# AY-Liu/Image-Editing-Framework

Hardware: AMD Instinct MI355X
Metric: denoising steps/sec (SD1.5 512x512 P2P edit step, UNet batch 4) (higher is better)
Workload: dtype f16x3; 1 GPU; sd15 UNet (859.5M params) P2P AttentionRefine edit step, 2 prompts x CFG = batch 4, 64x64 latents (512x512 px), 50-step DDIM, guidance 7.5, cross 0.8 / self 0.4, per-step null-text unconditional embeddings (P2P_NTI, edit_real.py); one independent edit per GPU; precision mode f16x3: fp32 storage; every contraction on split operands: hi + lo fp16 halves of each fp32 element, Ah Bh + Al Bh + Ah Bl =

## Files before the change

### image-editing-framework_amd/csrc/conv_halo_x3p.hip

```cpp
#include "x3p_common.h"

template <int N>
struct IntTag { static constexpr int value = N; };

template <bool UPS>
__global__ __launch_bounds__(768) void conv3x3_halo_x3p_kernel(const IefGemmX3pParams p) {
    constexpr int BM = 256, BN = 80, BK = XP_BK, NW = 8, NL = 4;
    constexpr int TM = 2, TN = 5;
    constexpr int WMAX = 64;
    constexpr int NPA = (BM + 2 * WMAX + 2 + 15) / 16;
    constexpr int APL = NPA * 1024;
    constexpr int AD = 2 * APL + 128;
    constexpr int ZA = 2 * APL;
    constexpr int NPB = BN / 16;
    constexpr int BPL = NPB * 1024, BBUF = 2 * BPL, NSB = 5;
    constexpr int BOFF = 2 * AD, DUMP = BOFF + NSB * BBUF;
    constexpr int LDS_BYTES = DUMP + 1024;
    constexpr int NU = 2 * NPA;
    constexpr int ATAPS = 5, APT = 3;
    static_assert(ATAPS * APT * NL >= NU && 3 * NL >= 2 * NPB, "loader schedule");
    static_assert(LDS_BYTES <= 160 * 1024, "LDS");
    __shared__ __attribute__((aligned(1024))) char smem[LDS_BYTES];

    const int tid = threadIdx.x, lane = tid & 63;
    const int wave = __builtin_amdgcn_readfirstlane(tid >> 6);
    const int tiles_n = (p.N + BN - 1) / BN, tiles_m = (p.M + BM - 1) / BM;
    const int lid = xcd_remap(blockIdx.x, gridDim.x);
    const int grp = lid / (XP_GROUP_M * tiles_n), within = lid - grp * (XP_GROUP_M * tiles_n);
    const int gsz = min(XP_GROUP_M, tiles_m - grp * XP_GROUP_M);
    const int tn = within / gsz, tm = grp * XP_GROUP_M + (within - tn * gsz);
    const int m0 = tm * BM, n0 = tn * BN;
    const int W = p.Wd, H = p.H;
    const int Ctot = p.C1 + p.C2;
    const char* __restrict__ zp = (const char*)p.zeros;
    const int Wi = W >> 1, Hi = H >> 1;
    const int ups_img = m0 / (H * W), ups_y0 = (m0 - ups_img * H * W) / W;
    const int ups_rel = ((ups_y0 - 1) >> 1) * Wi - 1;
    const int src_pixels = UPS ? p.batch_images * Hi * Wi : p.M;
    const int st_row0 = UPS ? ups_img * Hi * Wi + ups_rel : m0 - (W + 1);

    const int ncb = Ctot / BK;
    int cb_lo = 0, cb_hi = ncb;
    if (p.splits > 1) {
        const int per = (ncb + p.splits - 1) / p.splits;
        cb_lo = min(ncb, (int)blockIdx.y * per);
        cb_hi = min(ncb, cb_lo + per);
    }
    const int nblk = cb_hi - cb_lo, nsteps = nblk * 9;

    if (tid < 16) { ((float*)(smem + ZA))[tid] = 0.f; ((float*)(smem + ZA + AD))[tid] = 0.f; }
    asm volatile("s_waitcnt lgkmcnt(0)" ::: "memory");

    if (wave >= NW) {
        const int l = wave - NW;
        bool abl_prologue = true;
        const unsigned st_chunk = (unsigned)(XP_LANE_CHUNK(lane) * 16);
        const int ms_lane = st_row0 + (lane >> 2);
        const char* an_src = zp; long long an_pl = 0; unsigned an_cs = 0, an_c0 = 0; bool an_on = false;
        auto set_next_block = [&](int cb, bool on) {
            const bool first = cb * BK < p.C1;
            an_src = (const char*)(first ? p.A : p.A2);
            an_pl = (first ? p.planeA : p.planeA2) * 2;
            an_cs = (unsigned)(first ? p.C1 : p.C2);
            an_c0 = (unsigned)(first ? cb * BK : cb * BK - p.C1);
            an_on = on;
        };
        auto issue_a = [&](int u, int buf_off) {
            const bool exists = u < NU;
            const int pl = u >= NPA ? 1 : 0, q = u - pl * NPA;
            const int ms = ms_lane + 16 * q;
            const bool ok = exists && an_on && (unsigned)ms < (unsigned)src_pixels;
            const char* g = ok ? an_src + ((long long)pl * an_pl + (long long)((unsigned)ms * an_cs + an_c0) * 2 + st_chunk) : zp;
            if (!(XP_ABL & 1) || abl_prologue) glds16(g, (half_t*)(smem + (exists ? pl * AD + buf_off + q * 1024 : DUMP)));
        };
        const long long w_lane = (long long)(n0 + (lane >> 2)) * p.K * 2 + st_chunk;
        auto issue_b = [&](int cb, int tap, bool on, int slot_off) {
            const long long k0 = (long long)(tap * Ctot + cb * BK) * 2;
#pragma unroll
            for (int j = 0; j < 3; ++j) {
                const int v = l + NL * j;
                const bool exists = v < 2 * NPB;
                const int pl = v >= NPB ? 1 : 0, q = v - pl * NPB;
                const bool ok = exists && on && n0 + 16 * q + (lane >> 2) < p.N;
                const char* g = ok ? (const char*)p.W + ((long long)pl * p.planeW * 2 + w_lane + (long long)(16 * q) * p.K * 2 + k0) : zp;
                if (!(XP_ABL & 1) || abl_prologue) glds16(g, (half_t*)(smem + (exists ? BOFF + slot_off + pl * BPL + q * 1024 : DUMP)));
            }
        };
        auto n_issued = [](int tap) constexpr -> int { return 3 + (tap < ATAPS ? APT : 0); };
        if (nsteps > 0) {
            set_next_block(cb_lo, true);
            for (int u = l; u < ((NU + NL - 1) / NL) * NL; u += NL) issue_a(u, 0);
            issue_b(cb_lo, 0, true, 0);
            issue_b(cb_lo, 1, nsteps > 1, BBUF);
            issue_b(cb_lo, 2, nsteps > 2, 2 * BBUF);
            issue_b(cb_lo, 3, nsteps > 3, 3 * BBUF);
            asm volatile("s_waitcnt vmcnt(9)" ::: "memory");
            XP_BARRIER();
        }
        abl_prologue = false;
        int bs_prev = 4 * BBUF, bs = 0, bs_next = BBUF;
        for (int cbi = 0; cbi < nblk; ++cbi) {
            const int cb = cb_lo + cbi;
            const int abuf_n = APL - (cbi & 1) * APL;
            set_next_block(min(cb + 1, cb_hi - 1), cb + 1 < cb_hi);
            const int steps_left = nsteps - cbi * 9;
            auto one_step = [&](auto tap_tag) {
                constexpr int tap = decltype(tap_tag)::value;
                if (!(XP_ABL & 1)) asm volatile("s_waitcnt vmcnt(%0)" ::"n"(n_issued((tap + 8) % 9) + n_issued((tap + 7) % 9)) : "memory");
                XP_BARRIER();
                if constexpr (tap < ATAPS) {
#pragma unroll
                    for (int j = 0; j < APT; ++j) issue_a(APT * NL * tap + l + NL * j, abuf_n);
                }
                issue_b(cb + (tap + 4) / 9, (tap + 4) % 9, tap + 4 < steps_left, bs_prev);
                bs_prev = bs; bs = bs_next; bs_next = bs_next == (NSB - 1) * BBUF ? 0 : bs_next + BBUF;
            };
            one_step(IntTag<0>{}); one_step(IntTag<1>{}); one_step(IntTag<2>{});
            one_step(IntTag<3>{}); one_step(IntTag<4>{}); one_step(IntTag<5>{});
            one_step(IntTag<6>{}); one_step(IntTag<7>{}); one_step(IntTag<8>{});
        }
        asm volatile("s_waitcnt vmcnt(0)" ::: "memory");
        return;
    }

    const int fr = lane & 15, fq = lane >> 4;
    int a_row[TM], a_x[TM], a_y[TM];
    unsigned a_edge[TM];
#pragma unroll
    for (int i = 0; i < TM; ++i) {
        const int r = wave * 32 + i * 16 + fr, m = m0 + r;
        const int x = m % W, y = (m / W) % H;
        a_row[i] = r; a_x[i] = x; a_y[i] = y;
        a_edge[i] = (x == 0 ? 1u : 0u) | (x == W - 1 ? 2u : 0u) | (y == 0 ? 4u : 0u) | (y == H - 1 ? 8u : 0u) | (m >= p.M ? 16u : 0u);
    }
    int b_off[TN];
#pragma unroll
    for (int j = 0; j < TN; ++j) {
        const int row = j * 16 + fr;
        b_off[j] = BOFF + row * 64 + ((fq ^ xp_swz(row)) << 4);
    }
    f32x4 acc[TN][TM];
#pragma unroll
    for (int j = 0; j < TN; ++j)
#pragma unroll
        for (int i = 0; i < TM; ++i) acc[j][i] = f32x4{0.f, 0.f, 0.f, 0.f};

    auto a_addr = [&](int i, int abuf, int ky, int kx) -> int {
        const unsigned tmask = 16u | (kx == 0 ? 1u : 0u) | (kx == 2 ? 2u : 0u) | (ky == 0 ? 4u : 0u) | (ky == 2 ? 8u : 0u);
        int sr;
        if constexpr (UPS) sr = ((a_y[i] + ky - 1) >> 1) * Wi + ((a_x[i] + kx - 1) >> 1) - ups_rel;
        else sr = a_row[i] + ky * W + kx;
        const int ad = abuf + sr * 64 + ((fq ^ xp_swz(sr)) << 4);
        return (a_edge[i] & tmask) ? ZA : ad;
    };
    half8 ah[2][TM], al[2][TM], bh[TN], bl[TN];
    bool abl_read_done = false;
    auto read_a = [&](half8 (&h)[TM], half8 (&l)[TM], int abuf, int ky, int kx) {
        if ((XP_ABL & 2) && abl_read_done) return;
#pragma unroll
        for (int i = 0; i < TM; ++i) {
            const int ad = a_addr(i, abuf, ky, kx);
            h[i] = *(const half8*)(smem + ad);
            l[i] = *(const half8*)(smem + ad + AD);
        }
    };
    if (nsteps > 0) {
        XP_BARRIER();
        read_a(ah[0], al[0], 0, 0, 0);
#pragma unroll
        for (int j = 0; j < TN; ++j) { bh[j] = *(const half8*)(smem + b_off[j]); bl[j] = *(const half8*)(smem + b_off[j] + BPL); }
    }
    int bs_next = BBUF;
    auto one_step = [&](auto tap_tag, auto par_tag, int abuf, int abuf_n) {
        constexpr int tap = decltype(tap_tag)::value, PAR = decltype(par_tag)::value;
        XP_BARRIER();
        {
            constexpr int nky = tap == 8 ? 0 : (tap + 1) / 3, nkx = tap == 8 ? 0 : (tap + 1) % 3;
            read_a(ah[PAR ^ 1], al[PAR ^ 1], tap == 8 ? abuf_n : abuf, nky, nkx);
        }
#pragma unroll
        for (int j = 0; j < TN; ++j) {
#pragma unroll
            for (int i = 0; i < TM; ++i) {
                if (!(XP_ABL & 4)) {
                    acc[j][i] = __builtin_amdgcn_mfma_f32_16x16x32_f16(bl[j], ah[PAR][i], acc[j][i], 0, 0, 0);
                    acc[j][i] = __builtin_amdgcn_mfma_f32_16x16x32_f16(bh[j], al[PAR][i], acc[j][i], 0, 0, 0);
                }
                acc[j][i] = __builtin_amdgcn_mfma_f32_16x16x32_f16(bh[j], ah[PAR][i], acc[j][i], 0, 0, 0);
            }
            if (!(XP_ABL & 2)) {
                bh[j] = *(const half8*)(smem + bs_next + b_off[j]);
                bl[j] = *(const half8*)(smem + bs_next + b_off[j] + BPL);
            }
        }
        abl_read_done = true;
        bs_next = bs_next == (NSB - 1) * BBUF ? 0 : bs_next + BBUF;
    };
    for (int cbi = 0; cbi < nblk; cbi += 2) {
        {
            const int abuf = 0, abuf_n = APL;
            one_step(IntTag<0>{}, IntTag<0>{}, abuf, abuf_n); one_step(IntTag<1>{}, IntTag<1>{}, abuf, abuf_n);
            one_step(IntTag<2>{}, IntTag<0>{}, abuf, abuf_n); one_step(IntTag<3>{}, IntTag<1>{}, abuf, abuf_n);
            one_step(IntTag<4>{}, IntTag<0>{}, abuf, abuf_n); one_step(IntTag<5>{}, IntTag<1>{}, abuf, abuf_n);
            one_step(IntTag<6>{}, IntTag<0>{}, abuf, abuf_n); one_step(IntTag<7>{}, IntTag<1>{}, abuf, abuf_n);
            one_step(IntTag<8>{}, IntTag<0>{}, abuf, abuf_n);
        }
        if (cbi + 1 < nblk) {
            const int abuf = APL, abuf_n = 0;
            one_step(IntTag<0>{}, IntTag<1>{}, abuf, abuf_n); one_step(IntTag<1>{}, IntTag<0>{}, abuf, abuf_n);
            one_step(IntTag<2>{}, IntTag<1>{}, abuf, abuf_n); one_step(IntTag<3>{}, IntTag<0>{}, abuf, abuf_n);
            one_step(IntTag<4>{}, IntTag<1>{}, abuf, abuf_n); one_step(IntTag<5>{}, IntTag<0>{}, abuf, abuf_n);
            one_step(IntTag<6>{}, IntTag<1>{}, abuf, abuf_n); one_step(IntTag<7>{}, IntTag<0>{}, abuf, abuf_n);
            one_step(IntTag<8>{}, IntTag<1>{}, abuf, abuf_n);
        }
    }
    asm volatile("s_waitcnt lgkmcnt(0)" ::: "memory");

    const float inv = p.inv_scale;
    if (p.splits > 1) {
        float* slab = p.ws + (long long)blockIdx.y * p.M * p.N;
#pragma unroll
        for (int i = 0; i < TM; ++i) {
            const int m = m0 + wave * 32 + i * 16 + fr;
            if (m >= p.M) continue;
#pragma unroll
            for (int j = 0; j < TN; ++j) {
                const int n = n0 + j * 16 + 4 * fq;
                if (n < p.N) *(f32x4*)(slab + (long long)m * p.N + n) = acc[j][i] * inv;
            }
        }
        return;
    }
#pragma unroll
    for (int i = 0; i < TM; ++i) {
        const int m = m0 + wave * 32 + i * 16 + fr;
        if (m >= p.M) continue;
#pragma unroll
        for (int j = 0; j < TN; ++j) {
            const int n = n0 + j * 16 + 4 * fq;
            if (n < p.N) xp_store(p, acc[j][i] * inv, m, n);
        }
    }
}

int ief_conv_halo_x3p_dispatch(const IefGemmX3pParams& p, hipStream_t st) {
    if (!p.conv || p.stride != 1 || p.pad_hi_only || p.CE1 || p.CE2 || p.Wd < 2 || p.H < 2 || p.geglu) return IEF_ESHAPE;
    if (p.ups) {
        if (p.tile != 12 || p.Wd > 128 || (p.H * p.Wd) % 256 || 256 % p.Wd) return IEF_ESHAPE;
    } else if (p.tile != 11 || p.Wd > 64) return IEF_ESHAPE;
    const int ncb = (p.C1 + p.C2) / XP_BK;
    if (p.splits > ncb) return IEF_ESHAPE;
    const int tiles = ((p.M + 255) / 256) * ((p.N + 79) / 80);
    const int splits = p.splits > 1 ? p.splits : 1;
    if (p.ups) hipLaunchKernelGGL(conv3x3_halo_x3p_kernel<true>, dim3(tiles, splits), dim3(768), 0, st, p);
    else hipLaunchKernelGGL(conv3x3_halo_x3p_kernel<false>, dim3(tiles, splits), dim3(768), 0, st, p);
    IEF_LAUNCH_CHECK();
    return IEF_OK;
}
```

### image-editing-framework_amd/csrc/gemm_x3p.hip

```cpp
#include "ief_common.h"
#include "ief_params.h"
#include "x3_common.h"

#include "x3p_common.h"

template <int BM, int BN, int WAVES_M, int WAVES_N, int NS, int NL, bool CONV>
__global__ __launch_bounds__(64 * (WAVES_M * WAVES_N + NL)) void igemm_x3p_kernel(const IefGemmX3pParams p) {
    constexpr int BK = XP_BK;
    constexpr int NWC = WAVES_M * WAVES_N;
    constexpr int NSW = NL > 0 ? NL : NWC;
    constexpr int PA = BM / 16, PB = BN / 16;
    constexpr int P = 2 * (PA + PB);
    constexpr int G = (P + NSW - 1) / NSW;
    constexpr int WM = BM / WAVES_M, WN = BN / WAVES_N, TM = WM / 16, TN = WN / 16;
    constexpr int SLOT = P * 16 * BK;
    constexpr int DUMP = NS * SLOT;
    static_assert(BM % 16 == 0 && BN % 16 == 0 && WM % 16 == 0 && WN % 16 == 0, "tile");
    static_assert(NS >= 2 && NS <= 4, "ring depth");
    static_assert((NS * SLOT + 512) * 2 <= 160 * 1024, "LDS");
    __shared__ __attribute__((aligned(1024))) half_t smem[NS * SLOT + 512];

    const int tid = threadIdx.x, lane = tid & 63;
    const int wave = __builtin_amdgcn_readfirstlane(tid >> 6);
    const int wr = wave / WAVES_N, wc = wave % WAVES_N;
// ... 320 lines not shown
                }
            }
        }
        return;
    }
    const int slots_out = (p.N + WN - 1) / WN;
#pragma unroll
    for (int i = 0; i < TM; ++i) {
        const int m = m0 + wr * WM + i * 16 + fr;
        const bool mok = m < p.M;
        float mu = 0.f, rs = 1.f;
        if (p.rstat_in && mok) xp_ln_row(p, m, mu, rs);
        f32x4 vv[TN];
#pragma unroll
        for (int j = 0; j < TN; ++j) vv[j] = f32x4{0.f, 0.f, 0.f, 0.f};
#pragma unroll
        for (int P = 0; P < NP2; ++P) {
            const int n = cb + 32 * P + 8 * fq;
            if (!mok || n >= p.N) continue;
            f32x4 v0 = acc[2 * P][i] * inv, v1 = acc[2 * P + 1][i] * inv;
            if (n + 4 < p.N) {
                if (p.rstat_in) {
                    v0 = (v0 - *(const f32x4*)(p.colsum + n) * mu) * rs;
                    v1 = (v1 - *(const f32x4*)(p.colsum + n + 4) * mu) * rs;
                }
                xp_store8(p, v0, v1, m, n);
                vv[2 * P] = v0; vv[2 * P + 1] = v1;
            } else {
                if (p.rstat_in) v0 = (v0 - *(const f32x4*)(p.colsum + n) * mu) * rs;
                vv[2 * P] = xp_store(p, v0, m, n);
            }
        }
        if constexpr (TN & 1) {
            constexpr int j = TN - 1;
            const int n = cb + j * 16 + 4 * fq;
            if (mok && n < p.N) {
                f32x4 v = acc[j][i] * inv;
                if (p.rstat_in) v = (v - *(const f32x4*)(p.colsum + n) * mu) * rs;
                vv[j] = xp_store(p, v, m, n);
            }
        }
        if (p.rstat_out) {
            float sm, sq;
            xp_row_stats<TN>(vv, sm, sq);
            if (fq == 0 && mok && cb < p.N) {
                float* ro = p.rstat_out + ((long long)m * slots_out + cb / WN) * 2;
                ro[0] = sm; ro[1] = sq;
            }
        }
    }
}

__global__ __launch_bounds__(256) void x3p_reduce_kernel(const IefGemmX3pParams p) {
    const int N4 = p.N >> 2;
    const long long total = (long long)p.M * N4, slab = (long long)p.M * p.N;
    for (long long i = (long long)blockIdx.x * 256 + threadIdx.x; i < total; i += (long long)gridDim.x * 256) {
        const int m = (int)(i / N4), n = (int)(i - (long long)m * N4) * 4;
        const float* w = p.ws + (long long)m * p.N + n;
        f32x4 a = *(const f32x4*)w;
        int s = 1;
        for (; s + 3 < p.splits; s += 4) {
            f32x4 t[4];
#pragma unroll
            for (int u = 0; u < 4; ++u) t[u] = *(const f32x4*)(w + (s + u) * slab);
#pragma unroll
            for (int u = 0; u < 4; ++u) a += t[u];
        }
        for (; s < p.splits; ++s) a += *(const f32x4*)(w + s * slab);
        xp_store(p, a, m, n);
    }
}

__global__ __launch_bounds__(256) void x3_split_act_kernel(const float* __restrict__ x, half_t* __restrict__ planes, long long plane,
                                                           long long rows, int C4, int ldx, int ldp, float scale) {
    const long long total = rows * C4;
    for (long long i = (long long)blockIdx.x * 256 + threadIdx.x; i < total; i += (long long)gridDim.x * 256) {
        const long long r = i / C4;
        const int c = (int)(i - r * C4) * 4;
        half4 h, l;
        split4(*(const f32x4*)(x + r * ldx + c), scale, h, l);
        half_t* o = planes + r * ldp + c;
        *(half4*)o = h;
        *(half4*)(o + plane) = l;
    }
}
extern "C" int ief_x3_split_act(const float* x, ief_half* planes, long long plane, long long rows, int C, int ldx, int ldp, float scale,
                                void* stream) {
    if (!x || !planes) return IEF_EINVAL;
    if (rows <= 0 || C <= 0 || (C & 3) || (ldx & 3) || (ldp & 3) || (plane & 3) || !(scale > 0.f)) return IEF_ESHAPE;
    if (((uintptr_t)x & 15) || ((uintptr_t)planes & 7)) return IEF_EALIGN;
    long long grid = (rows * (C / 4) + 255) / 256;
    if (grid > 16384) grid = 16384;
    hipLaunchKernelGGL(x3_split_act_kernel, dim3((unsigned)grid), dim3(256), 0, (hipStream_t)stream, x, (half_t*)planes, plane, rows,
                       C / 4, ldx, ldp, scale);
    IEF_LAUNCH_CHECK();
    return IEF_OK;
}

extern "C" int ief_gemm_x3p_tile_bm(int tile) {
    switch (tile) {
        case 1: case 2: case 3: case 7: return 128;
        case 4: case 8: case 11: case 12: return 256;
        case 5: return 64;
        case 6: return 128;
        default: return 0;
    }
}
extern "C" int ief_gemm_x3p_tile_wn(int tile) { return tile == 6 ? 64 : tile == 8 ? 160 : 80; }
extern "C" int ief_gemm_x3p_tile_bn(int tile) {
    switch (tile) {
        case 1: case 2: case 4: case 5: case 7: return 160;
        case 3: case 11: case 12: return 80;
        case 6: return 64;
        case 8: return 320;
        default: return 0;
    }
}

template <int BM, int BN, int WAVES_M, int WAVES_N, int NS, int NL>
static int launch_x3p(const IefGemmX3pParams& p, hipStream_t st) {
    const int tiles = ((p.M + BM - 1) / BM) * ((p.N + BN - 1) / BN);
    const int splits = p.splits > 1 ? p.splits : 1;
    constexpr int NT = 64 * (WAVES_M * WAVES_N + NL);
    if (p.conv) hipLaunchKernelGGL((igemm_x3p_kernel<BM, BN, WAVES_M, WAVES_N, NS, NL, true>), dim3(tiles, splits), dim3(NT), 0, st, p);
    else hipLaunchKernelGGL((igemm_x3p_kernel<BM, BN, WAVES_M, WAVES_N, NS, NL, false>), dim3(tiles, splits), dim3(NT), 0, st, p);
    IEF_LAUNCH_CHECK();
    return IEF_OK;
}

int ief_conv_halo_x3p_dispatch(const IefGemmX3pParams& p, hipStream_t st);

extern "C" int ief_gemm_x3p(const IefGemmX3pParams* pp, void* stream) {
    if (!pp || !pp->A || !pp->W || !pp->zeros || (!pp->Out && !pp->OutP)) return IEF_EINVAL;
    IefGemmX3pParams p = *pp;
    if (p.M <= 0 || p.N <= 0 || p.K <= 0 || (p.K % XP_BK) || (p.N & 3)) return IEF_ESHAPE;
    if (p.rowvec && p.rows_per_batch <= 0) return IEF_ESHAPE;
    if (p.splits > 1 && (!p.ws || p.splits > 64 || p.geglu || p.rstat_out || p.cstat_out)) return IEF_EINVAL;
    if (!(p.inv_scale > 0.f)) return IEF_EINVAL;
    if ((p.ldw & 7) || (p.planeW & 7) || ((uintptr_t)p.W & 15)) return IEF_EALIGN;
    if (p.Out && ((p.ldo & 3) || ((uintptr_t)p.Out & 15))) return IEF_EALIGN;
    if (p.OutP && ((p.ldp & 3) || (p.planeO & 3) || ((uintptr_t)p.OutP & 7))) return IEF_EALIGN;
    if ((p.bias && ((uintptr_t)p.bias & 15)) || (p.rowvec && ((uintptr_t)p.rowvec & 15)) ||
        (p.residual && (((uintptr_t)p.residual & 15) || (p.ldr & 3)))) return IEF_EALIGN;
    if (p.geglu && ((p.N & 15) || p.residual || p.rowvec)) return IEF_EINVAL;
    if (p.rstat_out && (p.splits > 1 || p.geglu || p.tile == 11 || p.tile == 12 || (p.N % ief_gemm_x3p_tile_wn(p.tile)))) return IEF_EINVAL;
    if (p.rstat_in && (!p.colsum || p.rstat_slots <= 0 || p.rstat_cnt <= 0 || p.rstat_slots * p.rstat_cnt != p.K || p.splits > 1 ||
                       p.conv || !(p.ln_eps > 0.f) || ((uintptr_t)p.colsum & 15))) return IEF_EINVAL;
    if (p.conv) {
        if (p.C1 <= 0 || p.C2 < 0 || (p.C1 % XP_BK) || (p.C2 % XP_BK) || (p.CE1 % XP_BK) || (p.CE2 % XP_BK)) return IEF_ESHAPE;
        if ((p.C2 > 0 && !p.A2) || (p.CE1 > 0 && !p.E1) || (p.CE2 > 0 && !p.E2) || (p.CE2 > 0 && p.CE1 == 0)) return IEF_EINVAL;
        if (p.stride != 1 && p.stride != 2) return IEF_ESHAPE;
        if (p.ups != 0 && p.ups != 1) return IEF_ESHAPE;
        if (p.ups && ((p.H | p.Wd) & 1)) return IEF_ESHAPE;
        if ((p.CE1 + p.CE2) > 0 && (p.stride != 1 || p.ups)) return IEF_ESHAPE;
        if (p.K != 9 * (p.C1 + p.C2) + p.CE1 + p.CE2 || p.batch_images <= 0 || p.M != p.batch_images * p.Ho * p.Wo) return IEF_ESHAPE;
        const long long in_pix = (long long)p.batch_images * (p.H >> p.ups) * (p.Wd >> p.ups);
        const int cmax = p.C1 > p.C2 ? p.C1 : p.C2, emax = p.CE1 > p.CE2 ? p.CE1 : p.CE2;
        if (in_pix * cmax * 2 >= (1ll << 32) || (long long)p.M * emax * 2 >= (1ll << 32)) return IEF_ESHAPE;
        if (((uintptr_t)p.A & 15) || (p.planeA & 7) || (p.A2 && (((uintptr_t)p.A2 & 15) || (p.planeA2 & 7))) ||
            (p.E1 && (((uintptr_t)p.E1 & 15) || (p.planeE1 & 7))) || (p.E2 && (((uintptr_t)p.E2 & 15) || (p.planeE2 & 7)))) return IEF_EALIGN;
    } else {
        if ((p.lda & 7) || (p.planeA & 7) || ((uintptr_t)p.A & 15)) return IEF_EALIGN;
    }
    hipStream_t st = (hipStream_t)stream;
    int rc;
    switch (p.tile) {
        case 2: rc = launch_x3p<128, 160, 4, 2, 4, 4>(p, st); break;
        case 3: rc = launch_x3p<128, 80, 4, 1, 3, 0>(p, st); break;
        case 4: rc = launch_x3p<256, 160, 4, 2, 3, 0>(p, st); break;
        case 5: rc = launch_x3p<64, 160, 2, 2, 4, 0>(p, st); break;
        case 6: rc = launch_x3p<128, 64, 4, 1, 3, 0>(p, st); break;
        case 7: rc = launch_x3p<128, 160, 2, 2, 2, 0>(p, st); break;
        case 8: rc = launch_x3p<256, 320, 4, 2, 2, 0>(p, st); break;
        case 11: case 12: rc = ief_conv_halo_x3p_dispatch(p, st); break;
        case 1: default: rc = launch_x3p<128, 160, 4, 2, 4, 0>(p, st); break;
    }
    if (rc) return rc;
    if (p.splits > 1) {
        const long long total = (long long)p.M * (p.N / 4);
        int grid = (int)((total + 255) / 256);
        if (grid > 8192) grid = 8192;
        hipLaunchKernelGGL(x3p_reduce_kernel, dim3(grid), dim3(256), 0, st, p);
        IEF_LAUNCH_CHECK();
    }
    return IEF_OK;
}
```

### image-editing-framework_amd/planes.py

```python
import os
from ctypes import byref

import torch

from . import hip
from .hip import IefGemmX3pParams, _check, _dev32, _ptr, _stream, _Timed, _zeros

ACT_SCALE = 1.0
W_SCALE = hip.X3_SCALE_W


class Planes:
    __slots__ = ("t",)

    def __init__(self, t):
        if not (isinstance(t, torch.Tensor) and t.dtype == torch.float16 and t.dim() >= 2 and t.shape[0] == 2 and t.stride(-1) == 1):
            raise TypeError("Planes: expected an fp16 tensor [2, ...] with a contiguous last dimension")
        if not t.is_cuda:
            raise TypeError("Planes: device tensor expected (no CPU path)")
        self.t = t

    @staticmethod
    def empty(*shape, device):
        return Planes(torch.empty(2, *shape, dtype=torch.float16, device=device))
# ... 185 lines not shown
        if (Mp, Np) != (M, No):
            raise ValueError("x3p: out_planes shape mismatch")
        p.OutP, p.planeO, p.ldp = op.t.data_ptr(), op.plane, ldp
    return o32, op


def _ret(o32, op):
    if o32 is not None and op is not None:
        return o32, op
    return o32 if op is None else op


class RowStats:
    __slots__ = ("buf", "slots", "cnt")

    def __init__(self, buf, slots, cnt):
        self.buf, self.slots, self.cnt = buf, slots, cnt


class FoldedLN:
    __slots__ = ("w", "bias", "colsum", "eps")

    def __init__(self, w, bias, gamma, beta, eps):
        wf = (w * gamma[None, :]).contiguous()
        self.w = wf
        b = w @ beta
        self.bias = (b if bias is None else b + bias).contiguous()
        pl = weight_planes(wf)
        self.colsum = ((pl[0].float().sum(1) + pl[1].float().sum(1)) / W_SCALE).contiguous()
        self.eps = eps


LN_FOLD = os.environ.get("IEF_X3P_FOLD_LN", "0") == "1"


def gemm(a, w, bias=None, residual=None, rowvec=None, rows_per_batch=0, out=None, out_planes=None, out_scale=1.0,
         geglu=False, tile=0, splits=0, row_stats=False, ln=None):
    lib = hip.load()
    if not isinstance(a, Planes):
        raise TypeError("planes.gemm: a must be Planes")
    M, K, lda = a.rows_ld("a")
    N = w.shape[0]
    if w.dim() != 2 or w.shape[1] != K:
        raise ValueError(f"planes.gemm: K mismatch {tuple(w.shape)} vs {K}")
    wp = weight_planes(w)
    p = IefGemmX3pParams()
    p.A, p.planeA, p.lda = a.t.data_ptr(), a.plane, lda
    p.W, p.planeW, p.ldw = wp.data_ptr(), wp.stride(0), K
    No = N // 2 if geglu else N
    o32, op = _out_args(p, M, No, out, out_planes, a.device, a.shape[:-1])
    p.bias = _ptr(_dev32(bias, "bias")) if bias is not None else None
    if rowvec is not None:
        p.rowvec, p.rows_per_batch = _dev32(rowvec, "rowvec").data_ptr(), rows_per_batch
    if residual is not None:
        Mr, Nr, ldr = hip._rows_ld32(residual, "residual")
        if (Mr, Nr) != (M, N):
            raise ValueError("planes.gemm: residual shape mismatch")
        p.residual, p.ldr = residual.data_ptr(), ldr
    p.M, p.N, p.K = M, N, K
    p.out_scale, p.inv_scale = out_scale, 1.0 / (ACT_SCALE * W_SCALE)
    p.geglu, p.zeros = 1 if geglu else 0, _zeros(a.device)
    if tile:
        p.tile, p.splits = tile, max(1, splits)
    else:
        key = f"gemm|{M}|{N}|{K}" + ("|g" if geglu else "")
        if AUTOTUNE and key not in _plan_table() and not hip._capturing() and hip._prof is None:
            _autotune(key, candidate_plans(M, N, K, geglu=geglu),
                      lambda t, sp, wi: gemm(a, wi, bias=bias, residual=residual, rowvec=rowvec, rows_per_batch=rows_per_batch, out=out,
                                             out_planes=out_planes, out_scale=out_scale, geglu=geglu, tile=t, splits=sp), w)
        p.tile, p.splits = pick_plan(M, N, K, variant="|g" if geglu else "")
    if geglu or row_stats or ln is not None:
        p.splits = 1
    rs = None
    if row_stats:
        wn = lib.ief_gemm_x3p_tile_wn(p.tile)
        if N % wn:
            raise ValueError("planes.gemm: row statistics need N to be a multiple of the tile's wave width")
        rs = RowStats(torch.empty(M, N // wn, 2, dtype=torch.float32, device=a.device), N // wn, wn)
        p.rstat_out = rs.buf.data_ptr()
    if ln is not None:
        st, colsum, eps = ln
        if st.buf.shape[0] != M or st.slots * st.cnt != K or _dev32(colsum, "colsum").numel() != N:
            raise ValueError("planes.gemm: ln statistics / colsum do not match this launch")
        p.rstat_in, p.rstat_slots, p.rstat_cnt, p.colsum, p.ln_eps = st.buf.data_ptr(), st.slots, st.cnt, colsum.data_ptr(), eps
    ws = None
    if p.splits > 1:
        ws = torch.empty(p.splits * M * N, dtype=torch.float32, device=a.device)
        p.ws = ws.data_ptr()
    nbytes = 4.0 * (M * K + N * K + M * No * ((1 if o32 is not None else 0) + (1 if op is not None else 0)) + (M * N if residual is not None else 0))
    kn = f"igemm_x3p_kernel<false> t{p.tile}" + (f" {M}x{N}x{K} s{p.splits}" if hip.PROF_SHAPES else "")
    bm, bn = _TILES[p.tile]
    hip.note_staged(kn, 4.0 * K * (bm + bn) * -(-M // bm) * -(-N // bn))
    with _Timed(kn, 2.0 * M * N * K, nbytes):
        _check(lib.ief_gemm_x3p(byref(p), _stream()), "ief_gemm_x3p")
    r = _ret(o32, op)
    if row_stats:
        return (r + (rs,)) if isinstance(r, tuple) else (r, rs)
    return r


def conv3x3(x, w, bias=None, x2=None, stride=1, upsample=False, rowvec=None, residual=None, out=None, out_planes=None,
            extra=None, pad_hi_only=False, tile=0, splits=0):
    lib = hip.load()
    if not isinstance(x, Planes) or (x2 is not None and not isinstance(x2, Planes)):
        raise TypeError("planes.conv3x3: x / x2 must be Planes")
    if not x.is_contiguous() or (x2 is not None and not x2.is_contiguous()) or not w.is_contiguous():
        raise ValueError("planes.conv3x3: x, x2, w must be contiguous")
    B, Hp, Wp, C1 = x.shape
    C2 = 0 if x2 is None else x2.shape[-1]
    Cout = w.shape[0]
    e1 = e2 = None
    CE1 = CE2 = 0
    if extra is not None:
        e1, e2 = extra
        CE1 = e1.shape[-1]
        CE2 = 0 if e2 is None else e2.shape[-1]
        for e in (e1, e2):
            if e is not None and (not isinstance(e, Planes) or not e.is_contiguous() or tuple(e.shape[:3]) != (B, Hp, Wp)):
                raise ValueError("planes.conv3x3: extra sources must be contiguous NHWC Planes at the output resolution")
    K = 9 * (C1 + C2) + CE1 + CE2
    if w.numel() != Cout * K:
        raise ValueError(f"planes.conv3x3: weight {tuple(w.shape)} does not match K = {K}")
    H, Wd = (Hp * 2, Wp * 2) if upsample else (Hp, Wp)
    pad_total = 1 if pad_hi_only else 2
    Ho, Wo = (H + pad_total - 3) // stride + 1, (Wd + pad_total - 3) // stride + 1
    M = B * Ho * Wo
    wp = weight_planes(w)
    p = IefGemmX3pParams()
    p.A, p.planeA = x.t.data_ptr(), x.plane
    if x2 is not None:
        p.A2, p.planeA2 = x2.t.data_ptr(), x2.plane
    if e1 is not None:
        p.E1, p.planeE1 = e1.t.data_ptr(), e1.plane
    if e2 is not None:
        p.E2, p.planeE2 = e2.t.data_ptr(), e2.plane
    p.W, p.planeW, p.ldw = wp.data_ptr(), wp.stride(0), K
    o32, op = _out_args(p, M, Cout, out, out_planes, x.device, (B, Ho, Wo))
    p.bias = _ptr(_dev32(bias, "bias")) if bias is not None else None
    if rowvec is not None:
        _dev32(rowvec, "rowvec")
        if rowvec.dim() != 2 or rowvec.shape[1] != Cout or rowvec.shape[0] not in (1, B):
            raise ValueError("planes.conv3x3: rowvec must be [B, Cout] or [1, Cout]")
        p.rowvec = rowvec.data_ptr()
        p.rows_per_batch = Ho * Wo if rowvec.shape[0] == B and B > 1 else B * Ho * Wo
    if residual is not None:
        if tuple(hip._act32(residual, "residual").shape) != (B, Ho, Wo, Cout) or not residual.is_contiguous():
            raise ValueError("planes.conv3x3: residual must be contiguous fp32 [B, Ho, Wo, Cout]")
        p.residual, p.ldr = residual.data_ptr(), Cout
    p.M, p.N, p.K = M, Cout, K
    p.conv, p.H, p.Wd, p.C1, p.C2, p.Ho, p.Wo = 1, H, Wd, C1, C2, Ho, Wo
    p.stride, p.ups, p.batch_images, p.pad_hi_only = stride, 1 if upsample else 0, B, 1 if pad_hi_only else 0
    p.CE1, p.CE2 = CE1, CE2
    p.out_scale, p.inv_scale, p.zeros = 1.0, 1.0 / (ACT_SCALE * W_SCALE), _zeros(x.device)
    halo_ok = HALO and stride == 1 and not pad_hi_only and extra is None and Hp >= 2 and Cout % 80 == 0 and (
        (not upsample and 2 <= Wd <= 64) or (upsample and Wd <= 128 and (H * Wd) % 256 == 0 and 256 % Wd == 0))
    if tile:
        p.tile, p.splits = tile, max(1, splits)
    else:
        variant = ("|u" if upsample else "") + (f"|s{stride}" if stride != 1 else "") + ("|e" if extra is not None else "")
        key = f"conv|{M}|{Cout}|{K}{variant}"
        if AUTOTUNE and key not in _plan_table() and not hip._capturing() and hip._prof is None:
            _autotune(key, candidate_plans(M, Cout, K, conv=True, halo_ok=halo_ok, ncb=(C1 + C2) // 32),
                      lambda t, sp, wi: conv3x3(x, wi, bias, x2=x2, stride=stride, upsample=upsample, rowvec=rowvec, residual=residual,
                                                out=out, out_planes=out_planes, extra=extra, pad_hi_only=pad_hi_only, tile=t, splits=sp), w)
        hit = _plan_table().get(key)
        if hit is not None and (hit[0] not in (11, 12) or halo_ok):
            p.tile, p.splits = hit[0], hit[1]
        elif halo_ok:
            tiles, ncb = -(-M // 256) * (Cout // 80), (C1 + C2) // 32
            sp = 1
            while tiles * sp < 192 and sp * 2 <= ncb // 2 and sp < 16:
                sp *= 2
            p.tile, p.splits = 11, sp
        else:
            p.tile, p.splits = heuristic_plan(M, Cout, K, conv=True)
            if TILE_FORCE and TILE_FORCE < 10:
                p.tile = TILE_FORCE
    if p.tile in (11, 12):
        if not halo_ok:
            raise ValueError("planes.conv3x3: this geometry has no halo form (tile 11 / 12)")
        p.tile = 12 if upsample else 11
        p.splits = min(p.splits, (C1 + C2) // 32)
    ws = None
    if p.splits > 1:
        ws = torch.empty(p.splits * M * Cout, dtype=torch.float32, device=x.device)
        p.ws = ws.data_ptr()
    nbytes = 4.0 * (B * Hp * Wp * (C1 + C2) + M * (CE1 + CE2) + Cout * K + M * Cout * ((1 if o32 is not None else 0) + (1 if op is not None else 0) + (1 if residual is not None else 0)))
    kn = f"conv3x3_halo_x3p_kernel<{'true' if upsample else 'false'}>" if p.tile in (11, 12) else f"igemm_x3p_kernel<true> t{p.tile}"
    kn += f" {M}x{Cout}x{K} s{p.splits}" if hip.PROF_SHAPES else ""
    if p.tile in (11, 12):
        hip.note_staged(kn, 4.0 * (C1 + C2) * (9 * 80 + 256 + 2 * (Wd + 1)) * -(-M // 256) * -(-Cout // 80))
    else:
        bm, bn = _TILES[p.tile]
        hip.note_staged(kn, 4.0 * K * (bm + bn) * -(-M // bm) * -(-Cout // bn))
    with _Timed(kn, 2.0 * M * Cout * K, nbytes):
        _check(lib.ief_gemm_x3p(byref(p), _stream()), "ief_gemm_x3p (conv)")
    return _ret(o32, op)


GN_SMALL_ELEMS = int(os.environ.get("IEF_GN_SMALL_ELEMS", str(3 << 20)))
GN_REG_MAX_HW = int(os.environ.get("IEF_GN_REG_MAX_HW", "1024"))
HALO = os.environ.get("IEF_X3P_HALO", "1") == "1"
ENABLED = os.environ.get("IEF_X3P", "1") == "1"


def groupnorm(x, gamma, beta, groups, eps, silu=False, x2=None, out32=False):
    lib = hip.load()
    if not hip._act32(x, "x").is_contiguous() or (x2 is not None and not hip._act32(x2, "x2").is_contiguous()):
        raise ValueError("planes.groupnorm: inputs must be contiguous")
    B, C1 = x.shape[0], x.shape[-1]
    C2 = 0 if x2 is None else x2.shape[-1]
    HW = x.numel() // (B * C1)
    out = Planes.empty(*x.shape[:-1], C1 + C2, device=x.device)
    cpg = (C1 + C2) // groups
    if HW <= GN_REG_MAX_HW and lib.ief_groupnorm_reg_fits(C1, C2, HW, groups):
        o32 = torch.empty(*x.shape[:-1], C1 + C2, dtype=torch.float32, device=x.device) if out32 else None
        with _Timed("groupnorm_reg_kernel", 0.0, (12.0 if out32 else 8.0) * (x.numel() + (0 if x2 is None else x2.numel()))):
            _check(lib.ief_groupnorm_silu_reg(x.data_ptr(), _ptr(x2), C1, C2, _ptr(o32), out.t.data_ptr(), out.plane,
                                              _dev32(gamma, "gamma").data_ptr(), _dev32(beta, "beta").data_ptr(), B, HW, groups,
                                              eps, 1 if silu else 0, _stream()), "ief_groupnorm_silu_reg")
        return (out, o32) if out32 else out
    if not out32 and HW <= GN_REG_MAX_HW and B * HW * (C1 + C2) <= GN_SMALL_ELEMS and cpg % 2 == 0 and C1 % 2 == 0 and cpg // 2 <= 256:
        with _Timed("groupnorm_f32_kernel", 0.0, 12.0 * (x.numel() + (0 if x2 is None else x2.numel()))):
            _check(lib.ief_groupnorm_silu_x3p_small(x.data_ptr(), _ptr(x2), C1, C2, out.t.data_ptr(), out.plane,
                                                    _dev32(gamma, "gamma").data_ptr(), _dev32(beta, "beta").data_ptr(), B, HW, groups,
                                                    eps, 1 if silu else 0, _stream()), "ief_groupnorm_silu_x3p_small")
        return out
    o32 = torch.empty(*x.shape[:-1], C1 + C2, dtype=torch.float32, device=x.device) if out32 else None
    nws = lib.ief_groupnorm_f32_ws_floats(B, HW, C1 + C2)
    ws = torch.empty(nws, dtype=torch.float32, device=x.device)
    with _Timed("gn3_f32 (stats + finalize + apply)", 0.0, 12.0 * (x.numel() + (0 if x2 is None else x2.numel()))):
        _check(lib.ief_groupnorm_silu_x3p_ws(x.data_ptr(), _ptr(x2), C1, C2, _ptr(o32), out.t.data_ptr(), out.plane,
                                             _dev32(gamma, "gamma").data_ptr(), _dev32(beta, "beta").data_ptr(), B, HW, groups, eps,
                                             1 if silu else 0, ws.data_ptr(), nws, _stream()), "ief_groupnorm_silu_x3p_ws")
    return (out, o32) if out32 else out


def layernorm(x, gamma, beta, eps=1e-5):
    lib = hip.load()
    if not hip._act32(x, "x").is_contiguous():
        raise ValueError("planes.layernorm: x must be contiguous")
    C = x.shape[-1]
    out = Planes.empty(*x.shape, device=x.device)
    with _Timed("layernorm_f32_vec_kernel", 0.0, 8.0 * x.numel()):
        _check(lib.ief_layernorm_x3p(x.data_ptr(), out.t.data_ptr(), out.plane, _dev32(gamma, "gamma").data_ptr(),
                                     _dev32(beta, "beta").data_ptr(), x.numel() // C, C, eps, _stream()), "ief_layernorm_x3p")
    return out


def attn_out_args(p, B, N, C, device, out32=False):
    op = Planes.empty(B, N, C, device=device)
    p.OutP, p.planeO, p.sOPb, p.ldp = op.t.data_ptr(), op.plane, N * C, C
    o32 = None
    if out32:
        o32 = torch.empty(B, N, C, dtype=torch.float32, device=device)
        p.Out, p.sOb, p.ldo = o32.data_ptr(), N * C, C
    return op, o32


FLASH_PLANES = os.environ.get("IEF_X3P_FLASH", "1") == "1"
FLASH_PLANES_DIMS = (40, 64, 80)


def attn_flash(q, k, v, heads, scale, q_src=None, k_src=None, v_src=None, out=None, out_planes=True):
    lib = hip.load()
    for t, nm in ((q, "q"), (k, "k"), (v, "v")):
        if not isinstance(t, Planes) or t.dim() != 3:
            raise TypeError(f"planes.attn_flash: {nm} must be Planes [B, rows, heads*d]")
    B, N, C = q.shape
    L, d = k.shape[1], C // heads
    if d not in FLASH_PLANES_DIMS:
        raise ValueError(f"planes.attn_flash: head dim {d} has no planes instantiation")
    p = hip.IefAttnF32Params()
    for t, nm in ((q, "Q"), (k, "K"), (v, "V")):
        h_ = t.hi
        if h_.stride(2) != 1 or (h_.shape[0] > 1 and h_.stride(0) != h_.shape[1] * h_.stride(1)):
            raise ValueError("planes.attn_flash: operands must be [B, rows, heads*d] with batch stride rows * ld")
        setattr(p, nm + "p", h_.data_ptr())
        setattr(p, "plane" + nm, t.plane)
    p.ldq, p.ldk, p.ldv = q.hi.stride(1), k.hi.stride(1), v.hi.stride(1)
    p.sQb, p.sKb, p.sVb = q.hi.stride(0), k.hi.stride(0), v.hi.stride(0)
    p.B, p.heads, p.N, p.L, p.d, p.scale = B, heads, N, L, d, scale
    p.q_src, p.k_src, p.v_src = _ptr(hip._devi32(q_src, "q_src")), _ptr(hip._devi32(k_src, "k_src")), _ptr(hip._devi32(v_src, "v_src"))
    p.x3, p.zeros = 1, _zeros(q.device)
    op = None
    if out_planes:
        op, _ = attn_out_args(p, B, N, C, q.device)
    else:
        if out is None:
            out = torch.empty(B, N, C, dtype=torch.float32, device=q.device)
        p.Out, p.sOb, p.ldo = hip._act32(out, "out").data_ptr(), out.stride(0), out.stride(1)
    with _Timed(f"attn_flash_x3p_kernel<{d}>", 4.0 * B * heads * N * L * d, 4.0 * B * heads * d * (2 * N + 2 * L)):
        _check(lib.ief_attn_flash_f32(byref(p), _stream()), "ief_attn_flash_f32 (planes)")
    return op if out_planes else out
```

Before: 71.53 steps/s.

## Fuse 1x1 shortcut channels into halo conv3x3 kernel pipeline

The halo-staged conv3x3 kernel now accepts the extra 1x1 shortcut operands (E1/E2). After the last channel block it streams those K-blocks through the same loader and B-slot ring and accumulates them into the same tile. Before this, convs with a fused shortcut could not use the halo path and fell back to the generic implicit GEMM. The cost is more complex loader and consumer scheduling: a buffer handoff, an extra lgkmcnt wait, and split-K partitioning of the extra channels.

```diff
diff --git a/image-editing-framework_amd/csrc/conv_halo_x3p.hip b/image-editing-framework_amd/csrc/conv_halo_x3p.hip
--- a/image-editing-framework_amd/csrc/conv_halo_x3p.hip
+++ b/image-editing-framework_amd/csrc/conv_halo_x3p.hip
@@ -19,6 +19,8 @@
     constexpr int NU = 2 * NPA;
     constexpr int ATAPS = 5, APT = 3;
     static_assert(ATAPS * APT * NL >= NU && 3 * NL >= 2 * NPB, "loader schedule");
+    constexpr int XNP = BM / 16, XPL = XNP * 1024;
+    static_assert(3 * XPL <= 2 * APL && 2 * XNP <= ATAPS * APT * NL, "shortcut tiles");
     static_assert(LDS_BYTES <= 160 * 1024, "LDS");
     __shared__ __attribute__((aligned(1024))) char smem[LDS_BYTES];
 
@@ -47,6 +49,16 @@
         cb_hi = min(ncb, cb_lo + per);
     }
     const int nblk = cb_hi - cb_lo, nsteps = nblk * 9;
+    int e_lo = 0, e_hi = UPS ? 0 : (p.CE1 + p.CE2) / BK;
+    if (p.splits > 1) {
+        const int per = (ncb + p.splits - 1) / p.splits, ns = (ncb + per - 1) / per;
+        const int y = blockIdx.y, ne_all = e_hi;
+        e_lo = y < ns ? y * ne_all / ns : 0;
+        e_hi = y < ns ? (y + 1) * ne_all / ns : 0;
+    }
+    const int ne = e_hi - e_lo;
+    const int xoff0 = ((nblk - 1) & 1) ? 0 : 2 * XPL;
+    auto x_next = [](int xb) { return xb == 2 * XPL ? 0 : xb + XPL; };
 
     if (tid < 16) { ((float*)(smem + ZA))[tid] = 0.f; ((float*)(smem + ZA + AD))[tid] = 0.f; }
     asm volatile("s_waitcnt lgkmcnt(0)" ::: "memory");
@@ -55,27 +67,37 @@
         const int l = wave - NW;
         bool abl_prologue = true;
         const unsigned st_chunk = (unsigned)(XP_LANE_CHUNK(lane) * 16);
-        const int ms_lane = st_row0 + (lane >> 2);
         const char* an_src = zp; long long an_pl = 0; unsigned an_cs = 0, an_c0 = 0; bool an_on = false;
+        int an_np = NPA, an_r0 = st_row0 + (lane >> 2);
         auto set_next_block = [&](int cb, bool on) {
             const bool first = cb * BK < p.C1;
             an_src = (const char*)(first ? p.A : p.A2);
             an_pl = (first ? p.planeA : p.planeA2) * 2;
             an_cs = (unsigned)(first ? p.C1 : p.C2);
             an_c0 = (unsigned)(first ? cb * BK : cb * BK - p.C1);
-            an_on = on;
+            an_on = on; an_np = NPA; an_r0 = st_row0 + (lane >> 2);
+        };
+        auto set_next_extra = [&](int j) {
+            const int ch = (e_lo + j) * BK;
+            const bool first = ch < p.CE1;
+            an_src = (const char*)(first ? p.E1 : p.E2);
+            an_pl = (first ? p.planeE1 : p.planeE2) * 2;
+            an_cs = (unsigned)(first ? p.CE1 : p.CE2);
+            an_c0 = (unsigned)(first ? ch : ch - p.CE1);
+            an_on = j < ne; an_np = XNP; an_r0 = m0 + (lane >> 2);
         };
         auto issue_a = [&](int u, int buf_off) {
-            const bool exists = u < NU;
-            const int pl = u >= NPA ? 1 : 0, q = u - pl * NPA;
-            const int ms = ms_lane + 16 * q;
+            const int np = UPS ? NPA : an_np;
+            const bool exists = u < 2 * np;
+            const int pl = u >= np ? 1 : 0, q = u - pl * np;
+            const int ms = an_r0 + 16 * q;
             const bool ok = exists && an_on && (unsigned)ms < (unsigned)src_pixels;
             const char* g = ok ? an_src + ((long long)pl * an_pl + (long long)((unsigned)ms * an_cs + an_c0) * 2 + st_chunk) : zp;
             if (!(XP_ABL & 1) || abl_prologue) glds16(g, (half_t*)(smem + (exists ? pl * AD + buf_off + q * 1024 : DUMP)));
         };
         const long long w_lane = (long long)(n0 + (lane >> 2)) * p.K * 2 + st_chunk;
-        auto issue_b = [&](int cb, int tap, bool on, int slot_off) {
-            const long long k0 = (long long)(tap * Ctot + cb * BK) * 2;
+        auto issue_b = [&](int kk, bool on, int slot_off) {
+            const long long k0 = (long long)kk * 2;
 #pragma unroll
             for (int j = 0; j < 3; ++j) {
                 const int v = l + NL * j;
@@ -90,10 +112,10 @@
         if (nsteps > 0) {
             set_next_block(cb_lo, true);
             for (int u = l; u < ((NU + NL - 1) / NL) * NL; u += NL) issue_a(u, 0);
-            issue_b(cb_lo, 0, true, 0);
-            issue_b(cb_lo, 1, nsteps > 1, BBUF);
-            issue_b(cb_lo, 2, nsteps > 2, 2 * BBUF);
-            issue_b(cb_lo, 3, nsteps > 3, 3 * BBUF);
+            issue_b(cb_lo * BK, true, 0);
+            issue_b(Ctot + cb_lo * BK, true, BBUF);
+            issue_b(2 * Ctot + cb_lo * BK, true, 2 * BBUF);
+            issue_b(3 * Ctot + cb_lo * BK, true, 3 * BBUF);
             asm volatile("s_waitcnt vmcnt(9)" ::: "memory");
             XP_BARRIER();
         }
@@ -101,8 +123,10 @@
         int bs_prev = 4 * BBUF, bs = 0, bs_next = BBUF;
         for (int cbi = 0; cbi < nblk; ++cbi) {
             const int cb = cb_lo + cbi;
-            const int abuf_n = APL - (cbi & 1) * APL;
-            set_next_block(min(cb + 1, cb_hi - 1), cb + 1 < cb_hi);
+            const bool to_x = cb + 1 == cb_hi && ne > 0;
+            const int abuf_n = to_x ? xoff0 : APL - (cbi & 1) * APL;
+            if (to_x) set_next_extra(0);
+            else set_next_block(min(cb + 1, cb_hi - 1), cb + 1 < cb_hi);
             const int steps_left = nsteps - cbi * 9;
             auto one_step = [&](auto tap_tag) {
                 constexpr int tap = decltype(tap_tag)::value;
@@ -112,12 +136,29 @@
 #pragma unroll
                     for (int j = 0; j < APT; ++j) issue_a(APT * NL * tap + l + NL * j, abuf_n);
                 }
-                issue_b(cb + (tap + 4) / 9, (tap + 4) % 9, tap + 4 < steps_left, bs_prev);
+                const int past = tap + 4 - steps_left;
+                issue_b(past < 0 ? ((tap + 4) % 9) * Ctot + (cb + (tap + 4) / 9) * BK : 9 * Ctot + (e_lo + past) * BK, past < ne, bs_prev);
                 bs_prev = bs; bs = bs_next; bs_next = bs_next == (NSB - 1) * BBUF ? 0 : bs_next + BBUF;
             };
             one_step(IntTag<0>{}); one_step(IntTag<1>{}); one_step(IntTag<2>{});
             one_step(IntTag<3>{}); one_step(IntTag<4>{}); one_step(IntTag<5>{});
             one_step(IntTag<6>{}); one_step(IntTag<7>{}); one_step(IntTag<8>{});
+        }
+        if (ne > 0) {
+            int xb = x_next(xoff0);
+            set_next_extra(1);
+#pragma unroll
+            for (int i = 0; i < 2 * XNP / NL; ++i) issue_a(l + NL * i, xb);
+            for (int j = 0; j < ne; ++j) {
+                asm volatile("s_waitcnt vmcnt(%0)" ::"n"(3 + 2 * XNP / NL) : "memory");
+                XP_BARRIER();
+                xb = x_next(xb);
+                set_next_extra(j + 2);
+#pragma unroll
+                for (int i = 0; i < 2 * XNP / NL; ++i) issue_a(l + NL * i, xb);
+                issue_b(9 * Ctot + (e_lo + j + 4) * BK, j + 4 < ne, bs_prev);
+                bs_prev = bs; bs = bs_next; bs_next = bs_next == (NSB - 1) * BBUF ? 0 : bs_next + BBUF;
+            }
         }
         asm volatile("s_waitcnt vmcnt(0)" ::: "memory");
         return;
@@ -171,8 +212,13 @@
         for (int j = 0; j < TN; ++j) { bh[j] = *(const half8*)(smem + b_off[j]); bl[j] = *(const half8*)(smem + b_off[j] + BPL); }
     }
     int bs_next = BBUF;
+    const int cbi_hand = ne > 0 ? nblk - 1 : -1;
+    int cbi_cur = 0;
     auto one_step = [&](auto tap_tag, auto par_tag, int abuf, int abuf_n) {
         constexpr int tap = decltype(tap_tag)::value, PAR = decltype(par_tag)::value;
+        if constexpr (tap == 8) {
+            if (cbi_cur == cbi_hand) asm volatile("s_waitcnt lgkmcnt(0)" ::: "memory");
+        }
         XP_BARRIER();
         {
             constexpr int nky = tap == 8 ? 0 : (tap + 1) / 3, nkx = tap == 8 ? 0 : (tap + 1) % 3;
@@ -199,6 +245,7 @@
     for (int cbi = 0; cbi < nblk; cbi += 2) {
         {
             const int abuf = 0, abuf_n = APL;
+            cbi_cur = cbi;
             one_step(IntTag<0>{}, IntTag<0>{}, abuf, abuf_n); one_step(IntTag<1>{}, IntTag<1>{}, abuf, abuf_n);
             one_step(IntTag<2>{}, IntTag<0>{}, abuf, abuf_n); one_step(IntTag<3>{}, IntTag<1>{}, abuf, abuf_n);
             one_step(IntTag<4>{}, IntTag<0>{}, abuf, abuf_n); one_step(IntTag<5>{}, IntTag<1>{}, abuf, abuf_n);
@@ -207,6 +254,7 @@
         }
         if (cbi + 1 < nblk) {
             const int abuf = APL, abuf_n = 0;
+            cbi_cur = cbi + 1;
             one_step(IntTag<0>{}, IntTag<1>{}, abuf, abuf_n); one_step(IntTag<1>{}, IntTag<0>{}, abuf, abuf_n);
             one_step(IntTag<2>{}, IntTag<1>{}, abuf, abuf_n); one_step(IntTag<3>{}, IntTag<0>{}, abuf, abuf_n);
             one_step(IntTag<4>{}, IntTag<1>{}, abuf, abuf_n); one_step(IntTag<5>{}, IntTag<0>{}, abuf, abuf_n);
@@ -214,6 +262,33 @@
             one_step(IntTag<8>{}, IntTag<1>{}, abuf, abuf_n);
         }
     }
+    if (ne > 0) {
+        int x_off[TM];
+#pragma unroll
+        for (int i = 0; i < TM; ++i) x_off[i] = a_row[i] * 64 + ((fq ^ xp_swz(a_row[i])) << 4);
+        int xb = xoff0;
+        for (int j = 0; j < ne; ++j) {
+            XP_BARRIER();
+#pragma unroll
+            for (int i = 0; i < TM; ++i) {
+                ah[0][i] = *(const half8*)(smem + xb + x_off[i]);
+                al[0][i] = *(const half8*)(smem + xb + x_off[i] + AD);
+            }
+#pragma unroll
+            for (int jn = 0; jn < TN; ++jn) {
+#pragma unroll
+                for (int i = 0; i < TM; ++i) {
+                    acc[jn][i] = __builtin_amdgcn_mfma_f32_16x16x32_f16(bl[jn], ah[0][i], acc[jn][i], 0, 0, 0);
+                    acc[jn][i] = __builtin_amdgcn_mfma_f32_16x16x32_f16(bh[jn], al[0][i], acc[jn][i], 0, 0, 0);
+                    acc[jn][i] = __builtin_amdgcn_mfma_f32_16x16x32_f16(bh[jn], ah[0][i], acc[jn][i], 0, 0, 0);
+                }
+                bh[jn] = *(const half8*)(smem + bs_next + b_off[jn]);
+                bl[jn] = *(const half8*)(smem + bs_next + b_off[jn] + BPL);
+            }
+            bs_next = bs_next == (NSB - 1) * BBUF ? 0 : bs_next + BBUF;
+            xb = x_next(xb);
+        }
+    }
     asm volatile("s_waitcnt lgkmcnt(0)" ::: "memory");
 
     const float inv = p.inv_scale;
@@ -244,7 +319,8 @@
 }
 
 int ief_conv_halo_x3p_dispatch(const IefGemmX3pParams& p, hipStream_t st) {
-    if (!p.conv || p.stride != 1 || p.pad_hi_only || p.CE1 || p.CE2 || p.Wd < 2 || p.H < 2 || p.geglu) return IEF_ESHAPE;
+    if (!p.conv || p.stride != 1 || p.pad_hi_only || p.Wd < 2 || p.H < 2 || p.geglu) return IEF_ESHAPE;
+    if (p.ups && (p.CE1 || p.CE2)) return IEF_EINVAL;
     if (p.ups) {
         if (p.tile != 12 || p.Wd > 128 || (p.H * p.Wd) % 256 || 256 % p.Wd) return IEF_ESHAPE;
     } else if (p.tile != 11 || p.Wd > 64) return IEF_ESHAPE;
diff --git a/image-editing-framework_amd/csrc/gemm_x3p.hip b/image-editing-framework_amd/csrc/gemm_x3p.hip
--- a/image-editing-framework_amd/csrc/gemm_x3p.hip
+++ b/image-editing-framework_amd/csrc/gemm_x3p.hip
@@ -496,7 +496,8 @@
         if (p.stride != 1 && p.stride != 2) return IEF_ESHAPE;
         if (p.ups != 0 && p.ups != 1) return IEF_ESHAPE;
         if (p.ups && ((p.H | p.Wd) & 1)) return IEF_ESHAPE;
-        if ((p.CE1 + p.CE2) > 0 && (p.stride != 1 || p.ups)) return IEF_ESHAPE;
+        if ((p.CE1 + p.CE2) > 0 && p.ups) return IEF_EINVAL;
+        if ((p.CE1 + p.CE2) > 0 && p.stride != 1) return IEF_ESHAPE;
         if (p.K != 9 * (p.C1 + p.C2) + p.CE1 + p.CE2 || p.batch_images <= 0 || p.M != p.batch_images * p.Ho * p.Wo) return IEF_ESHAPE;
         const long long in_pix = (long long)p.batch_images * (p.H >> p.ups) * (p.Wd >> p.ups);
         const int cmax = p.C1 > p.C2 ? p.C1 : p.C2, emax = p.CE1 > p.CE2 ? p.CE1 : p.CE2;
diff --git a/image-editing-framework_amd/planes.py b/image-editing-framework_amd/planes.py
--- a/image-editing-framework_amd/planes.py
+++ b/image-editing-framework_amd/planes.py
@@ -361,8 +361,8 @@
     p.stride, p.ups, p.batch_images, p.pad_hi_only = stride, 1 if upsample else 0, B, 1 if pad_hi_only else 0
     p.CE1, p.CE2 = CE1, CE2
     p.out_scale, p.inv_scale, p.zeros = 1.0, 1.0 / (ACT_SCALE * W_SCALE), _zeros(x.device)
-    halo_ok = HALO and stride == 1 and not pad_hi_only and extra is None and Hp >= 2 and Cout % 80 == 0 and (
-        (not upsample and 2 <= Wd <= 64) or (upsample and Wd <= 128 and (H * Wd) % 256 == 0 and 256 % Wd == 0))
+    halo_ok = HALO and stride == 1 and not pad_hi_only and Hp >= 2 and Cout % 80 == 0 and (
+        (not upsample and 2 <= Wd <= 64) or (upsample and extra is None and Wd <= 128 and (H * Wd) % 256 == 0 and 256 % Wd == 0))
     if tile:
         p.tile, p.splits = tile, max(1, splits)
     else:
@@ -398,7 +398,7 @@
     kn = f"conv3x3_halo_x3p_kernel<{'true' if upsample else 'false'}>" if p.tile in (11, 12) else f"igemm_x3p_kernel<true> t{p.tile}"
     kn += f" {M}x{Cout}x{K} s{p.splits}" if hip.PROF_SHAPES else ""
     if p.tile in (11, 12):
-        hip.note_staged(kn, 4.0 * (C1 + C2) * (9 * 80 + 256 + 2 * (Wd + 1)) * -(-M // 256) * -(-Cout // 80))
+        hip.note_staged(kn, 4.0 * ((C1 + C2) * (9 * 80 + 256 + 2 * (Wd + 1)) + (CE1 + CE2) * (80 + 256)) * -(-M // 256) * -(-Cout // 80))
     else:
         bm, bn = _TILES[p.tile]
         hip.note_staged(kn, 4.0 * K * (bm + bn) * -(-M // bm) * -(-Cout // bn))
```

Result: no change. 71.66 steps/s (median of 4 runs) (+0.2%).
